# Graph-Machine-Learning-Group/sgp

Hardware: AMD Instinct MI355X
Metric: encoded node-steps/sec (higher is better)
Workload: dtype f32 (hop products: operands as fp16 hi + lo pairs, three 16-bit MFMA terms per product, fp32 accumulation -- agrees with fp32 to ~1e-7 of the operand scale; reservoir: recurrent products: state (|h| <= 1, x 2^14) and W_hh (per-row power-of-two scale) as two fp16 pieces (22 bits), hi*hi + hi*lo + lo*

## Files before the change

include/sgp_amd.h:

```cpp
#ifndef SGP_AMD_H
#define SGP_AMD_H

#include <stdint.h>

#ifdef __cplusplus
extern "C" {
#endif

#define SGP_ABI_VERSION 3

#define SGP_EINVAL   (-1)
#define SGP_EUNSUP   (-2)
#define SGP_ENOMEM   (-3)

#define SGP_ACT_TANH      0
#define SGP_ACT_RELU      1
#define SGP_ACT_SELF_NORM 2
#define SGP_ACT_IDENTITY  3
#define SGP_ACT_TANH_REL  4

typedef void* sgp_stream_t;

int sgp_abi_version(void);
const char* sgp_last_error(void);
// ... 8 lines not shown
                     float* Y, int64_t y_row_stride, int64_t y_batch_stride,
                     int32_t n_rows, int32_t n_cols, int32_t batch, int32_t feat,
                     const int32_t* pred, int32_t run_if, sgp_stream_t stream);

int sgp_spmm_tiled_f32(const int32_t* tile_row_ptr, const int32_t* uptr, const int32_t* ucol,
                       const int32_t* erow, const uint16_t* ecol, const float* eval,
                       int32_t tile_rows, int32_t n_tiles,
                       int32_t max_union, int32_t max_row_edges,
                       const float* X, int64_t x_row_stride, int64_t x_batch_stride,
                       const float* X_halo, int64_t xh_row_stride, int64_t xh_batch_stride,
                       int32_t n_own,
                       float* Y, int64_t y_row_stride, int64_t y_batch_stride,
                       int32_t n_rows, int32_t n_cols, int32_t batch, int32_t feat,
                       const int32_t* pred, int32_t run_if, sgp_stream_t stream);
int sgp_spmm_res_f32(const int32_t* uptr, const int32_t* ucol, const int32_t* usplit,
                     const int32_t* gptr, const int32_t* gsup, const int32_t* gidx, const float* gw,
                     const int32_t* rowmap,
                     int32_t n_tiles, int32_t max_union, int32_t max_tile_quads,
                     const float* X, int64_t x_row_stride, int64_t x_batch_stride,
                     const float* X_halo, int64_t xh_row_stride, int64_t xh_batch_stride,
                     int32_t n_own,
                     float* Y, int64_t y_row_stride, int64_t y_batch_stride,
                     int32_t n_rows, int32_t n_cols, int32_t batch, int32_t feat,
                     const int32_t* pred, int32_t run_if, sgp_stream_t stream);
int32_t sgp_spmm_res_max_union(void);
int32_t sgp_spmm_res_max_quads(void);
int sgp_spmm_res_tune(int32_t cfg);

int sgp_spmm_mix_f32(const int32_t* uptr, const int32_t* ucol, const int32_t* usplit,
                     const int32_t* gptr, const int32_t* gsup, const int32_t* gidx, const float* gw,
                     const int32_t* rowmap,
                     const int32_t* dptr, const int32_t* didx, const float* dw,
                     int32_t n_tiles, int32_t max_union, int32_t max_dense,
                     const float* X, int64_t x_row_stride, int64_t x_batch_stride,
                     const float* X_halo, int64_t xh_row_stride, int64_t xh_batch_stride,
                     int32_t n_own,
                     float* Y, int64_t y_row_stride, int64_t y_batch_stride,
                     int32_t n_rows, int32_t n_cols, int32_t batch, int32_t feat,
                     const int32_t* pred, int32_t run_if, sgp_stream_t stream);
int32_t sgp_spmm_mix_max_union(void);
int32_t sgp_spmm_mix_max_dense(int32_t halo);

int sgp_abs_max_f32(const float* X, int64_t x_row_stride, int64_t x_batch_stride,
                    int32_t n_rows, int32_t batch, int32_t feat, float* out, sgp_stream_t stream);


int sgp_col_stats_f32(const float* X, int64_t x_row_stride, int64_t x_batch_stride,
                      int32_t n_rows, int32_t batch, int32_t feat, int32_t t_stride, int32_t r_stride, int32_t accumulate,
                      float* stats, sgp_stream_t stream);

int sgp_split_prepare_f32(const float* stats, double n_samples, double s_eff, int32_t full,
                          const float* bound_in, float bound_scalar, float norm_inf, int32_t feat,
                          float* x_tab, float* bound_out, int32_t* flag, sgp_stream_t stream);

int sgp_spmm_split_f32(const int32_t* hdr, const int32_t* rowid, const int32_t* ucol, const void* afr,
                       const int32_t* adr, const float* rinv, int32_t n_tiles,
                       const float* X, int64_t x_row_stride, int64_t x_batch_stride,
                       const float* X_halo, int64_t xh_row_stride, int64_t xh_batch_stride, int32_t n_own,
                       float* Y, int64_t y_row_stride, int64_t y_batch_stride,
                       int32_t n_rows, int32_t n_cols, int32_t batch, int32_t feat,
                       const float* x_tab, int32_t accumulate, int32_t t_chunk, const int32_t* pred, int32_t run_if, sgp_stream_t stream);
int32_t sgp_spmm_split_chunks(void);
int32_t sgp_spmm_split_max_union(void);
int32_t sgp_spmm_split_waves(void);
int32_t sgp_spmm_split_rows_per_wave(void);
int32_t sgp_spmm_split_max_feat(void);

int sgp_spmm_split_banded_f32(const int32_t* hdr, const int32_t* rowid, const int32_t* ucol, const void* afr,
                              const int32_t* adr, const float* rinv, int32_t n_tiles,
                              const float* X, int64_t x_row_stride, int64_t x_batch_stride,
                              const float* X_halo, int64_t xh_row_stride, int64_t xh_batch_stride, int32_t n_own,
                              float* Y, int64_t y_row_stride, int64_t y_batch_stride,
                              int32_t n_rows, int32_t n_cols, int32_t batch, int32_t feat,
                              const float* x_tab, int32_t accumulate, int32_t t_chunk,
                              int32_t walk, const int32_t* band_first, int32_t n_bands,
                              const int32_t* pred, int32_t run_if, sgp_stream_t stream);

int sgp_spmm_split_wide_f32(const int32_t* hdr, const int32_t* rowid, const int32_t* ucol, const void* afr,
                            const int32_t* adr, const float* rinv, int32_t n_tiles,
                            const float* X, int64_t x_row_stride, int64_t x_batch_stride,
                            const float* X_halo, int64_t xh_row_stride, int64_t xh_batch_stride, int32_t n_own,
                            float* Y, int64_t y_row_stride, int64_t y_batch_stride,
                            int32_t n_rows, int32_t n_cols, int32_t batch, int32_t feat,
                            const float* x_tab, int32_t accumulate, int32_t t_chunk, const int32_t* pred, int32_t run_if, sgp_stream_t stream);
int sgp_spmm_split_wide_banded_f32(const int32_t* hdr, const int32_t* rowid, const int32_t* ucol, const void* afr,
                                   const int32_t* adr, const float* rinv, int32_t n_tiles,
                                   const float* X, int64_t x_row_stride, int64_t x_batch_stride,
                                   const float* X_halo, int64_t xh_row_stride, int64_t xh_batch_stride, int32_t n_own,
                                   float* Y, int64_t y_row_stride, int64_t y_batch_stride,
                                   int32_t n_rows, int32_t n_cols, int32_t batch, int32_t feat,
                                   const float* x_tab, int32_t accumulate, int32_t t_chunk,
                                   int32_t walk, const int32_t* band_first, int32_t n_bands,
                                   const int32_t* pred, int32_t run_if, sgp_stream_t stream);
int32_t sgp_spmm_split_wide_chunks(void);
int32_t sgp_spmm_split_wide_max_union(void);
int32_t sgp_spmm_split_wide_waves(void);
int32_t sgp_spmm_split_wide_rows_per_wave(void);
int32_t sgp_spmm_split_wide_max_feat(void);

int64_t sgp_split_plan_deal(const int64_t* rowptr, const int64_t* col, int64_t nnz, int64_t n_rows, int64_t n_cols,
                            const int64_t* order, int64_t n_order,
                            int32_t waves, int32_t chunks, int32_t max_union, int32_t rows_per_wave,
                            int64_t* wave_of_row, int64_t* slot_of_row, int64_t* tile_of_wave, int64_t* rows_of_wave);
int sgp_split_plan_fill(const int64_t* rowptr, const int64_t* col, const float* val, int64_t nnz, int64_t n_rows, int64_t n_cols,
                        const int64_t* wave_of_row, const int64_t* slot_of_row, const int64_t* tile_of_wave,
                        const int64_t* rows_of_wave, int64_t n_waves, int64_t n_tiles,
// ... 366 lines not shown
```

sgp_amd/csrc/split_prepare.hip:

```cpp
#include "common.h"

namespace {

__global__ __launch_bounds__(256) void col_stats_kernel(const float* x, long long xrs, long long xbs, int n_rows,
                                                        int t_stride, int feat, unsigned* amax, float* ssq) {
    const int q = feat >> 2;
    const int rpi = 256 / q;
    const int r0 = threadIdx.x / q, c = threadIdx.x - r0 * q;
    const float* xb = x + (long long)blockIdx.y * t_stride * xbs;
    unsigned m[4] = {0, 0, 0, 0};
    float s[4] = {0.f, 0.f, 0.f, 0.f};
    if (r0 < rpi) {
        auto take = [&](const float4 v) {
            m[0] = max(m[0], __float_as_uint(fabsf(v.x))); s[0] = fmaf(v.x, v.x, s[0]);
            m[1] = max(m[1], __float_as_uint(fabsf(v.y))); s[1] = fmaf(v.y, v.y, s[1]);
            m[2] = max(m[2], __float_as_uint(fabsf(v.z))); s[2] = fmaf(v.z, v.z, s[2]);
            m[3] = max(m[3], __float_as_uint(fabsf(v.w))); s[3] = fmaf(v.w, v.w, s[3]);
        };
        const long long step = (long long)gridDim.x * rpi;
        long long r = (long long)blockIdx.x * rpi + r0;
        for (; r + 3 * step < n_rows; r += 4 * step) {
            const float4 v0 = *(const float4*)(xb + r * xrs + 4 * c);
            const float4 v1 = *(const float4*)(xb + (r + step) * xrs + 4 * c);
            const float4 v2 = *(const float4*)(xb + (r + 2 * step) * xrs + 4 * c);
            const float4 v3 = *(const float4*)(xb + (r + 3 * step) * xrs + 4 * c);
            take(v0); take(v1); take(v2); take(v3);
        }
        for (; r < n_rows; r += step) take(*(const float4*)(xb + r * xrs + 4 * c));
    }
    __shared__ unsigned pm[256][4];
    __shared__ float ps[256][4];
#pragma unroll
    for (int i = 0; i < 4; ++i) { pm[threadIdx.x][i] = m[i]; ps[threadIdx.x][i] = s[i]; }
    __syncthreads();
    if (threadIdx.x < q) {
        for (int r = 1; r < rpi; ++r) {
#pragma unroll
            for (int i = 0; i < 4; ++i) { m[i] = max(m[i], pm[r * q + c][i]); s[i] += ps[r * q + c][i]; }
        }
#pragma unroll
        for (int i = 0; i < 4; ++i) { atomicMax(amax + 4 * c + i, m[i]); atomicAdd(ssq + 4 * c + i, s[i]); }
    }
}

struct PrepArgs {
    const unsigned* amax; const float* ssq;
    double n_samples, s_eff;
    int full;
    const float* bound_in; float bound_scalar;
    float norm_inf;
    int feat;
    float* tab; float* bound_out; int* flag;
};

__global__ __launch_bounds__(256) void split_prepare_kernel(PrepArgs a) {
    int ok = 1;
    for (int c = threadIdx.x; c < a.feat; c += 256) {
        float b;
        const float mx = a.amax ? __uint_as_float(a.amax[c]) : 0.f;
        if (a.bound_in) b = a.bound_in[c];
        else if (a.bound_scalar > 0.f) b = a.bound_scalar;
        else b = mx;
        if (a.amax && !(mx <= b)) ok = 0;
        float scale = 1.f, inv = 1.f;
        if (!(b >= 0.f) || !(b < __builtin_inff())) { ok = 0; b = __builtin_inff(); }
        else if (b > 0.f) {
            int k;
            const float mant = frexpf(b, &k);
            int e = (mant == 0.5f ? 15 : 14) - k;
            e = min(126, max(-126, e));
            scale = ldexpf(1.f, e); inv = ldexpf(1.f, -e);
            if (a.amax) {
                const double rms = sqrt((double)a.ssq[c] / a.n_samples);
                if (!((double)b * sqrt(a.s_eff) <= 65536.0 * rms)) ok = 0;
            }
        }
        a.tab[c] = scale; a.tab[a.feat + c] = inv;
        if (a.bound_out) a.bound_out[c] = b * a.norm_inf * (1.f + 1e-6f);
    }
    ok = __syncthreads_and(ok);
    if (threadIdx.x == 0) a.flag[0] = ok;
}

}

extern "C" {

int sgp_col_stats_f32(const float* X, int64_t x_row_stride, int64_t x_batch_stride,
                      int32_t n_rows, int32_t batch, int32_t feat, int32_t t_stride, int32_t r_stride, int32_t accumulate,
                      float* stats, sgp_stream_t stream) {
    SGP_REQUIRE(X && stats, "sgp_col_stats_f32: null pointer");
    SGP_REQUIRE(n_rows >= 0 && batch >= 0 && feat > 0 && feat % 4 == 0 && feat <= 1024 && t_stride >= 1 && r_stride >= 1,
                "sgp_col_stats_f32: feat must be a multiple of 4 up to 1024, strides >= 1");
    n_rows = (n_rows + r_stride - 1) / r_stride;
    x_row_stride *= r_stride;
    SGP_REQUIRE(sgp::aligned16(X) && x_row_stride % 4 == 0 && x_batch_stride % 4 == 0, "sgp_col_stats_f32: rows must be 16-byte aligned");
    hipStream_t s = (hipStream_t)stream;
    if (!accumulate) {
        hipError_t e = hipMemsetAsync(stats, 0, 2 * (size_t)feat * sizeof(float), s);
        if (e != hipSuccess) return sgp::fail((int)e, "sgp_col_stats_f32: memset: %s", hipGetErrorString(e));
    }
    if (n_rows == 0 || batch == 0) return 0;
    const int ns = (batch + t_stride - 1) / t_stride;
    SGP_REQUIRE(ns <= 65535, "sgp_col_stats_f32: more than 65535 sampled steps");
    const int rpi = 256 / (feat / 4);
    long long gx = ((long long)n_rows + rpi - 1) / rpi;
    const long long cap = 512 / ns > 0 ? 512 / ns : 1;
    if (gx > cap) gx = cap;
    hipLaunchKernelGGL(col_stats_kernel, dim3((unsigned)gx, (unsigned)ns), dim3(256), 0, s,
                       X, (long long)x_row_stride, (long long)x_batch_stride, n_rows, t_stride, feat,
                       (unsigned*)stats, stats + feat);
    return sgp::check_launch("col_stats");
}

int sgp_split_prepare_f32(const float* stats, double n_samples, double s_eff, int32_t full,
                          const float* bound_in, float bound_scalar, float norm_inf, int32_t feat,
                          float* x_tab, float* bound_out, int32_t* flag, sgp_stream_t stream) {
    SGP_REQUIRE(x_tab && flag, "sgp_split_prepare_f32: null pointer");
    SGP_REQUIRE(feat > 0 && feat <= 1024, "sgp_split_prepare_f32: feat out of range");
    SGP_REQUIRE(stats || bound_in || bound_scalar > 0.f, "sgp_split_prepare_f32: neither statistics nor a bound");
    SGP_REQUIRE(!stats || (n_samples >= 1.0 && s_eff >= 1.0), "sgp_split_prepare_f32: statistics need their sample counts");
    SGP_REQUIRE(stats || full == 0, "sgp_split_prepare_f32: full = 1 needs statistics");
    SGP_REQUIRE(bound_in || bound_scalar > 0.f || full, "sgp_split_prepare_f32: a measured bound needs statistics of every row");
    PrepArgs a;
    a.amax = (const unsigned*)stats; a.ssq = stats ? stats + feat : nullptr;
    a.n_samples = n_samples; a.s_eff = s_eff; a.full = full;
    a.bound_in = bound_in; a.bound_scalar = bound_scalar; a.norm_inf = norm_inf; a.feat = feat;
    a.tab = x_tab; a.bound_out = bound_out; a.flag = flag;
    hipLaunchKernelGGL(split_prepare_kernel, dim3(1), dim3(256), 0, (hipStream_t)stream, a);
    return sgp::check_launch("split_prepare");
}

}
```

sgp_amd/csrc/spmm.hip:

```cpp
#include "common.h"
#include <stdlib.h>

using sgp::f32x4;

namespace {

constexpr int kWave = 64;

__device__ __forceinline__ f32x4 ld4(const float* p) { return *reinterpret_cast<const f32x4*>(p); }
__device__ __forceinline__ void st4(float* p, f32x4 v) { *reinterpret_cast<f32x4*>(p) = v; }

struct Src {
    const float* x;  long long xrs, xbs;
    const float* xh; long long xhrs, xhbs;
    int n_own;
    const int* pred; int pred_want;
    __device__ __forceinline__ bool skip() const { return pred != nullptr && pred[0] != pred_want; }
    __device__ __forceinline__ const float* row(int b, int c) const {
        return (c < n_own) ? x + (long long)b * xbs + (long long)c * xrs
                           : xh + (long long)b * xhbs + (long long)(c - n_own) * xhrs;
    }
};

template <int LPR, int TB>
// ... 12 lines not shown
    for (int i = 0; i < TB; ++i) acc[i] = f32x4{0.f, 0.f, 0.f, 0.f};

    const int e1 = rowptr[row + 1];
    for (int e = rowptr[row] + g; e < e1; e += G) {
        const int c = col[e];
        const float v = val[e];
#pragma unroll
        for (int i = 0; i < TB; ++i) {
            if (fok && b0 + i < batch) {
                const f32x4 xv = ld4(src.row(b0 + i, c) + f0);
                acc[i] += v * xv;
            }
        }
    }
#pragma unroll
    for (int i = 0; i < TB; ++i) {
#pragma unroll
        for (int off = LPR; off < kWave; off <<= 1) {
            acc[i].x += __shfl_xor(acc[i].x, off);
            acc[i].y += __shfl_xor(acc[i].y, off);
            acc[i].z += __shfl_xor(acc[i].z, off);
            acc[i].w += __shfl_xor(acc[i].w, off);
        }
    }
#pragma unroll
    for (int i = 0; i < TB; ++i) {
        if (fok && b0 + i < batch && g == (i % G))
            st4(Y + (long long)(b0 + i) * ybs + (long long)row * yrs + f0, acc[i]);
    }
}

template <int LPR, int TB>
__global__ __launch_bounds__(256) void spmm_csr_rows(
        const int* __restrict__ rowptr, const int* __restrict__ col, const float* __restrict__ val,
        Src src, float* __restrict__ Y, long long yrs, long long ybs,
        int n_rows, int batch, int feat) {
    const int row = blockIdx.x * 4 + (threadIdx.x >> 6);
    if (row >= n_rows || src.skip()) return;
    csr_rows_body<LPR, TB>(rowptr, col, val, src, Y, yrs, ybs, batch, feat, row, blockIdx.y * TB);
}

template <int LPR, int TB>
__global__ __launch_bounds__(256) void spmm_csr_rows_strided(
        const int* __restrict__ rowptr, const int* __restrict__ col, const float* __restrict__ val,
        Src src, float* __restrict__ Y, long long yrs, long long ybs,
        int n_rows, int batch, int feat) {
    if (src.skip()) return;
    const int n_rb = (n_rows + 3) / 4, n_bb = (batch + TB - 1) / TB;
    for (int bb = blockIdx.y; bb < n_bb; bb += gridDim.y)
        for (int rb = blockIdx.x; rb < n_rb; rb += gridDim.x) {
            const int row = rb * 4 + (threadIdx.x >> 6);
            if (row < n_rows) csr_rows_body<LPR, TB>(rowptr, col, val, src, Y, yrs, ybs, batch, feat, row, bb * TB);
        }
}

__global__ __launch_bounds__(256) void spmm_csr_scalar(
        const int* __restrict__ rowptr, const int* __restrict__ col, const float* __restrict__ val,
        Src src, float* __restrict__ Y, long long yrs, long long ybs,
        int n_rows, int batch, int feat) {
    const int lane = threadIdx.x & 63;
    const int row = blockIdx.x * 4 + (threadIdx.x >> 6);
    const int b = blockIdx.y;
    if (row >= n_rows || src.skip()) return;
    const int e0 = rowptr[row], e1 = rowptr[row + 1];
    for (int f = lane; f < feat; f += kWave) {
        float acc = 0.f;
        for (int e = e0; e < e1; ++e) acc += val[e] * src.row(b, col[e])[f];
        Y[(long long)b * ybs + (long long)row * yrs + f] = acc;
    }
}

template <int S>
__device__ __forceinline__ int ror_i(int v) {
    if constexpr (S == 0) return v;
    else return __builtin_amdgcn_update_dpp(0, v, 0x120 + S, 0xf, 0xf, true);
}
template <int S>
__device__ __forceinline__ float ror_f(float v) {
    return __int_as_float(ror_i<S>(__float_as_int(v)));
}

template <int S0>
__device__ __forceinline__ void edge_half(const char* lds, int off, float w, int li16, f32x4& acc) {
    int ad[8];
    float wv[8];
    f32x4 xv[8];
#define SGP_ROT(i) ad[i] = ror_i<S0 + i>(off) + li16; wv[i] = ror_f<S0 + i>(w);
    SGP_ROT(0) SGP_ROT(1) SGP_ROT(2) SGP_ROT(3) SGP_ROT(4) SGP_ROT(5) SGP_ROT(6) SGP_ROT(7)
#undef SGP_ROT
#pragma unroll
    for (int i = 0; i < 8; ++i) xv[i] = *reinterpret_cast<const f32x4*>(lds + ad[i]);
#pragma unroll
    for (int i = 0; i < 8; ++i) acc += wv[i] * xv[i];
}

#define SGP_FMAC_ROR(S, ACC, W, X)                                                              \
    asm("v_fmac_f32_dpp %0, %1, %2 row_ror:" #S " row_mask:0xf bank_mask:0xf" : "+v"(ACC) : "v"(W), "v"(X))
#define SGP_STEP_ROR(S, I)                                                                      \
    SGP_FMAC_ROR(S, acc.x, w, xv[I].x); SGP_FMAC_ROR(S, acc.y, w, xv[I].y);                     \
    SGP_FMAC_ROR(S, acc.z, w, xv[I].z); SGP_FMAC_ROR(S, acc.w, w, xv[I].w);
template <int S0, int ABL = 0>
__device__ __forceinline__ void edge_half_dpp(const char* lds, int off, float w, int li16, f32x4& acc) {
    int ad[8];
    f32x4 xv[8];
#define SGP_ROT(i) ad[i] = ror_i<S0 + i>(off) + li16;
    SGP_ROT(0) SGP_ROT(1) SGP_ROT(2) SGP_ROT(3) SGP_ROT(4) SGP_ROT(5) SGP_ROT(6) SGP_ROT(7)
// ... 265 lines not shown
int sgp_spmm_tiled_form(int32_t tile_rows, int32_t max_row_edges, int32_t* rows_per_group, int32_t* batches) {
    SGP_REQUIRE(tile_rows > 0 && max_row_edges >= 0 && max_row_edges % 16 == 0, "sgp_spmm_tiled_form: bad size");
    if (tile_rows > sgp_spmm_tiled_max_tile_rows() || max_row_edges > sgp_spmm_tiled_max_row_edges())
        return sgp::fail(SGP_EUNSUP, "sgp_spmm_tiled_f32: tile_rows=%d / max_row_edges=%d out of range",
                         tile_rows, max_row_edges);
    int rpg = (tile_rows + kTiledGroups - 1) / kTiledGroups;
    rpg = rpg <= 2 ? rpg : (rpg <= 4 ? 4 : 6);
    const int nb = (rpg > 2 && max_row_edges <= 16) ? 1 : (max_row_edges <= 32 ? 2 : 8);
    if (rows_per_group) *rows_per_group = rpg;
    if (batches) *batches = nb;
    if (nb == 8 && rpg != 1)
        return sgp::fail(SGP_EUNSUP, "spmm_tiled: no kernel for rows/group=%d batches=%d", rpg, nb);
    return 0;
}

int32_t sgp_spmm_csr_form(int32_t feat, int32_t aligned, int32_t predicated) {
    (void)predicated;
    if (feat <= 0 || feat % 4 != 0 || !aligned) return 0;
    if (feat >= 256 || feat % 256 == 0) return 64;
    return feat > 64 ? 32 : feat > 32 ? 16 : feat > 16 ? 8 : 4;
}

int sgp_spmm_csr_f32(const int32_t* rowptr, const int32_t* col, const float* val,
                     const float* X, int64_t xrs, int64_t xbs,
                     const float* Xh, int64_t xhrs, int64_t xhbs, int32_t n_own,
                     float* Y, int64_t yrs, int64_t ybs,
                     int32_t n_rows, int32_t n_cols, int32_t batch, int32_t feat,
                     const int32_t* pred, int32_t run_if, sgp_stream_t stream) {
    const sgp::Predicate pr{pred, run_if};
    SGP_REQUIRE(rowptr && col && val && X && Y, "sgp_spmm_csr_f32: null pointer");
    SGP_REQUIRE(n_rows >= 0 && n_cols >= 0 && batch >= 0 && feat >= 0, "sgp_spmm_csr_f32: negative size");
    SGP_REQUIRE(Xh != nullptr || n_own >= n_cols, "sgp_spmm_csr_f32: n_own < n_cols needs X_halo");
    if (n_rows == 0 || batch == 0 || feat == 0) return 0;
    hipStream_t s = (hipStream_t)stream;
    Src src{X, xrs, xbs, Xh ? Xh : X, xhrs, xhbs, Xh ? n_own : 0x7fffffff, pr.flag, pr.want};
    const bool vec = feat % 4 == 0 && xrs % 4 == 0 && xbs % 4 == 0 && yrs % 4 == 0 && ybs % 4 == 0 &&
                     sgp::aligned16(X) && sgp::aligned16(Y) &&
                     (!Xh || (xhrs % 4 == 0 && xhbs % 4 == 0 && sgp::aligned16(Xh)));
    const unsigned gx = (n_rows + 3) / 4;
    if (sgp_spmm_csr_form(feat, vec, pr.flag != nullptr) == 0) {
        SGP_REQUIRE(batch <= 65535, "sgp_spmm_csr_f32: scalar path supports batch <= 65535");
        hipLaunchKernelGGL(spmm_csr_scalar, dim3(gx, batch), dim3(256), 0, s,
                           rowptr, col, val, src, Y, yrs, ybs, n_rows, batch, feat);
        return sgp::check_launch("spmm_csr_scalar");
    }
    constexpr int TB = 4;
    const unsigned gy = (batch + TB - 1) / TB;
    SGP_REQUIRE(gy <= 65535, "sgp_spmm_csr_f32: batch too large for one launch (chunk it)");
    const bool bounded = pr.flag != nullptr;
#define SGP_ROWS(LPR)                                                                          \
    do {                                                                                       \
        if (bounded)                                                                           \
            hipLaunchKernelGGL((spmm_csr_rows_strided<LPR, TB>),                               \
                               dim3(gx < 2048u ? gx : 2048u, gy < 8u ? gy : 8u, (feat + 4 * LPR - 1) / (4 * LPR)), \
                               dim3(256), 0, s, rowptr, col, val, src, Y, yrs, ybs, n_rows, batch, feat);          \
        else                                                                                   \
            hipLaunchKernelGGL((spmm_csr_rows<LPR, TB>), dim3(gx, gy, (feat + 4 * LPR - 1) / (4 * LPR)), \
                               dim3(256), 0, s, rowptr, col, val, src, Y, yrs, ybs, n_rows, batch, feat);  \
    } while (0)
    switch (sgp_spmm_csr_form(feat, 1, bounded)) {
        case 64: SGP_ROWS(64); break;
        case 32: SGP_ROWS(32); break;
        case 16: SGP_ROWS(16); break;
        case 8: SGP_ROWS(8); break;
        default: SGP_ROWS(4); break;
    }
#undef SGP_ROWS
    return sgp::check_launch("spmm_csr_rows");
}

int sgp_spmm_tiled_f32(const int32_t* trow, const int32_t* uptr, const int32_t* ucol,
                       const int32_t* erow, const uint16_t* ecol, const float* eval,
                       int32_t tile_rows, int32_t n_tiles, int32_t max_union, int32_t max_row_edges,
                       const float* X, int64_t xrs, int64_t xbs,
                       const float* Xh, int64_t xhrs, int64_t xhbs, int32_t n_own,
                       float* Y, int64_t yrs, int64_t ybs,
                       int32_t n_rows, int32_t n_cols, int32_t batch, int32_t feat,
                       const int32_t* pred, int32_t run_if, sgp_stream_t stream) {
    const sgp::Predicate pr{pred, run_if};
    SGP_REQUIRE(trow && uptr && ucol && erow && ecol && eval && X && Y, "sgp_spmm_tiled_f32: null pointer");
    SGP_REQUIRE(tile_rows > 0 && n_tiles >= 0 && n_rows >= 0 && batch >= 0 && max_union >= 0 &&
                max_row_edges >= 0 && max_row_edges % 16 == 0, "sgp_spmm_tiled_f32: bad size");
    SGP_REQUIRE((long long)tile_rows * n_tiles >= n_rows, "sgp_spmm_tiled_f32: tiles do not cover rows");
    {
        const long long own = Xh ? n_own : n_cols, far = Xh ? n_cols - n_own : 0;
        SGP_REQUIRE(n_cols >= 0 && own >= 0 && far >= 0 && own * xrs < (1ll << 31) && far * xhrs < (1ll << 31),
                    "sgp_spmm_tiled_f32: row offsets exceed 32 bits (use sgp_spmm_csr_f32)");
    }
    if (n_rows == 0 || batch == 0 || feat == 0) return 0;
    if (feat % 64 != 0)
        return sgp::fail(SGP_EUNSUP, "sgp_spmm_tiled_f32: feat=%d is not a multiple of 64", feat);
    if (max_union > kTiledCapacity)
        return sgp::fail(SGP_EUNSUP, "sgp_spmm_tiled_f32: a tile references %d distinct rows, LDS stage holds %d",
                         max_union, kTiledCapacity);
    int32_t rpg = 0, nb = 0;
    const int form_rc = sgp_spmm_tiled_form(tile_rows, max_row_edges, &rpg, &nb);
    if (form_rc && rpg == 0) return form_rc;
    SGP_REQUIRE(xrs % 4 == 0 && xbs % 4 == 0 && yrs % 4 == 0 && ybs % 4 == 0 &&
                sgp::aligned16(X) && sgp::aligned16(Y) &&
                (!Xh || (xhrs % 4 == 0 && xhbs % 4 == 0 && sgp::aligned16(Xh))),
                "sgp_spmm_tiled_f32: strides/pointers must be 16-byte aligned");
    TiledArgs a;
    a.trow = trow; a.uptr = uptr; a.ucol = ucol; a.erow = erow; a.ecol = ecol; a.eval = eval;
    a.tile_rows = tile_rows; a.n_tiles = n_tiles;
    a.src = Src{X, xrs, xbs, Xh ? Xh : X, xhrs, xhbs, Xh ? n_own : 0x7fffffff, pr.flag, pr.want};
    a.Y = Y; a.yrs = yrs; a.ybs = ybs;
    a.n_rows = n_rows; a.batch = batch; a.feat = feat;
// ... 14 lines not shown
```

sgp_amd/hip.py:

```python
import ctypes
import json
import os
import subprocess

import torch

_CSRC = os.path.join(os.path.dirname(os.path.abspath(__file__)), "csrc")
LIB_PATH = os.environ.get("SGP_AMD_LIB") or os.path.join(_CSRC, "libsgp_amd.so")

c_i32, c_i64, c_f32, c_f64, c_p = (ctypes.c_int32, ctypes.c_int64,
                                   ctypes.c_float, ctypes.c_double,
                                   ctypes.c_void_p)
c_u64 = ctypes.c_uint64

SIGNATURES = {
    "sgp_abi_version": (ctypes.c_int, []),
    "sgp_last_error": (ctypes.c_char_p, []),
    "sgp_build_arch": (ctypes.c_char_p, []),
    "sgp_tune_value": (c_i64, [ctypes.c_char_p, c_i64]),
    "sgp_spmm_csr_f32": (ctypes.c_int, [c_p, c_p, c_p,
                                        c_p, c_i64, c_i64,
                                        c_p, c_i64, c_i64, c_i32,
                                        c_p, c_i64, c_i64,
                                        c_i32, c_i32, c_i32, c_i32, c_p, c_i32, c_p]),
# ... 54 lines not shown
                                               c_i32, c_i32, c_i32, c_i32, c_i32, c_p]),
    "sgp_reservoir_fused_sums_f32": (ctypes.c_int, [c_p, c_i64, c_i64,
                                                    c_p, c_p, c_p,
                                                    c_p, c_i32,
                                                    c_p, c_i64, c_i64,
                                                    c_p, c_p, c_p,
                                                    c_i32, c_i32, c_i32, c_i32, c_i32, c_p]),
    "sgp_reservoir_window_supported": (c_i32, [c_i32, c_i32, c_i32]),
    "sgp_reservoir_window_workspace_bytes": (c_i64, [c_i32, c_i32, c_i32, c_i32, c_i64]),
    "sgp_reservoir_window_f32": (ctypes.c_int, [c_p, c_i64, c_i64, c_i64, c_i32,
                                                c_p, c_i64, c_i64, c_i64, c_i32,
                                                c_p,
                                                c_p, c_p, c_p, c_p, c_i32,
                                                c_p, c_p, c_i64,
                                                c_p, c_i32,
                                                c_i32, c_i32, c_i32, c_i32, c_i32, c_p]),
    "sgp_gesn_workspace_bytes": (c_i64, [c_i32, c_i32, c_i32]),
    "sgp_gesn_tune": (ctypes.c_int, [c_i32]),
    "sgp_gesn_f32": (ctypes.c_int, [c_p, c_p, c_p, c_p, c_i64, c_i64, c_p, c_p, c_p, c_p, c_i32,
                                    c_p, c_i64, c_i64, c_p, c_p,
                                    c_i32, c_i32, c_i32, c_i32, c_i32, c_p]),
    "sgp_gemm_nt_f32": (ctypes.c_int, [c_p, c_i64, c_p, c_i64, c_p, c_p, c_i64,
                                       c_i32, c_i32, c_i32, c_p]),
    "sgp_gesn_update_f32": (ctypes.c_int, [c_p, c_p, c_p, c_p, c_p, c_p, c_f64, c_i32,
                                           c_p, c_p, c_i64, c_i32, c_i32, c_p]),
    "sgp_node_mean_bcast_f32": (ctypes.c_int, [c_p, c_i64, c_i64,
                                               c_p, c_i64, c_i64, c_p,
                                               c_i32, c_i32, c_i32, c_p]),
    "sgp_bcast_rows_f32": (ctypes.c_int, [c_p, c_f32, c_p, c_i64, c_i64,
                                          c_i32, c_i32, c_i32, c_p]),
    "sgp_copy_rows_f32": (ctypes.c_int, [c_p, c_i64, c_i64, c_p, c_i64, c_i64,
                                         c_i32, c_i32, c_i32, c_p]),
    "sgp_gather_rows_f32": (ctypes.c_int, [c_p, c_i64, c_i64, c_p, c_p, c_i32,
                                           c_p, c_i64, c_i64, c_i32, c_i32, c_p]),
    "sgp_grouped_linear_packed_floats": (c_i64, [c_i32, c_i32, c_i32]),
    "sgp_grouped_linear_pack_f32": (ctypes.c_int, [c_p, c_p, c_i32, c_i32, c_i32, c_p]),
    "sgp_grouped_linear_f32": (ctypes.c_int, [c_p, c_i64, c_i64, c_p, c_p, c_p, c_p, c_i32,
                                              c_p, c_i64, c_i32, c_i32, c_i32, c_i32, c_p]),
    "sgp_grouped_linear_fwd_f32": (ctypes.c_int, [c_p, c_i64, c_i64, c_p, c_p, c_p, c_p, c_i32,
                                                  c_p, c_i64, c_p, c_f64, c_u64,
                                                  c_i32, c_i32, c_i32, c_i32, c_p]),
    "sgp_grouped_linear_dact_f32": (ctypes.c_int, [c_p, c_i64, c_p, c_i32, c_f64, c_u64, c_p, c_i64, c_i32, c_p]),
    "sgp_grouped_linear_transpose_f32": (ctypes.c_int, [c_p, c_p, c_i32, c_i32, c_i32, c_p]),
    "sgp_grouped_linear_wgrad_f32": (ctypes.c_int, [c_p, c_i64, c_i64, c_p, c_p, c_p, c_p,
                                                    c_i32, c_i32, c_i32, c_i32, c_p]),
    "sgp_grouped_linear_form": (ctypes.c_int, [c_i32, c_i32, c_i64, c_i64, c_i32, c_p, c_p]),
    "sgp_grouped_linear_wgrad_form": (ctypes.c_int, [c_i32, c_i32, c_i32, c_i32, c_p, c_p]),
    "sgp_abs_max_f32": (ctypes.c_int, [c_p, c_i64, c_i64, c_i32, c_i32, c_i32, c_p, c_p]),
    "sgp_spmm_split_f32": (ctypes.c_int, [c_p, c_p, c_p, c_p, c_p, c_p, c_i32, c_p, c_i64, c_i64,
                                          c_p, c_i64, c_i64, c_i32, c_p, c_i64, c_i64,
                                          c_i32, c_i32, c_i32, c_i32, c_p, c_i32, c_i32, c_p, c_i32, c_p]),
    "sgp_col_stats_f32": (ctypes.c_int, [c_p, c_i64, c_i64, c_i32, c_i32, c_i32, c_i32, c_i32, c_i32, c_p, c_p]),
    "sgp_split_prepare_f32": (ctypes.c_int, [c_p, c_f64, c_f64, c_i32, c_p, c_f32, c_f32, c_i32, c_p, c_p, c_p, c_p]),
    "sgp_spmm_split_wide_f32": (ctypes.c_int, [c_p, c_p, c_p, c_p, c_p, c_p, c_i32, c_p, c_i64, c_i64,
                                               c_p, c_i64, c_i64, c_i32, c_p, c_i64, c_i64,
                                               c_i32, c_i32, c_i32, c_i32, c_p, c_i32, c_i32, c_p, c_i32, c_p]),
    "sgp_spmm_split_wide_chunks": (c_i32, []),
    "sgp_spmm_split_wide_max_union": (c_i32, []),
    "sgp_spmm_split_wide_waves": (c_i32, []),
    "sgp_spmm_split_wide_rows_per_wave": (c_i32, []),
    "sgp_spmm_split_wide_max_feat": (c_i32, []),
    "sgp_spmm_split_chunks": (c_i32, []),
    "sgp_spmm_split_max_union": (c_i32, []),
    "sgp_spmm_split_waves": (c_i32, []),
    "sgp_spmm_split_rows_per_wave": (c_i32, []),
    "sgp_spmm_split_max_feat": (c_i32, []),
    "sgp_split_plan_deal": (c_i64, [c_p, c_p, c_i64, c_i64, c_i64, c_p, c_i64, c_i32, c_i32, c_i32, c_i32, c_p, c_p, c_p, c_p]),
    "sgp_split_plan_fill": (ctypes.c_int, [c_p, c_p, c_p, c_i64, c_i64, c_i64, c_p, c_p, c_p, c_p, c_i64, c_i64,
                                           c_i32, c_i32, c_i32, c_p, c_p, c_p, c_p, c_p, c_p, c_p, c_i32]),
    "sgp_split_plan_bands": (c_i64, [c_p, c_i64, c_i32, c_i64, c_i64, c_p]),
    "sgp_spmm_split_banded_f32": (ctypes.c_int, [c_p, c_p, c_p, c_p, c_p, c_p, c_i32, c_p, c_i64, c_i64,
                                                 c_p, c_i64, c_i64, c_i32, c_p, c_i64, c_i64,
                                                 c_i32, c_i32, c_i32, c_i32, c_p, c_i32, c_i32, c_i32, c_p, c_i32,
                                                 c_p, c_i32, c_p]),
    "sgp_spmm_split_wide_banded_f32": (ctypes.c_int, [c_p, c_p, c_p, c_p, c_p, c_p, c_i32, c_p, c_i64, c_i64,
                                                      c_p, c_i64, c_i64, c_i32, c_p, c_i64, c_i64,
                                                      c_i32, c_i32, c_i32, c_i32, c_p, c_i32, c_i32, c_i32, c_p, c_i32,
                                                      c_p, c_i32, c_p]),
    "sgp_spmm_colblock_f32": (ctypes.c_int, [c_p, c_p, c_p, c_i32, c_i32, c_p, c_i64, c_i64,
                                             c_p, c_i64, c_i64, c_i32, c_p, c_i64, c_i64,
                                             c_i32, c_i32, c_i32, c_i32, c_p, c_i32, c_p]),
    "sgp_spmm_colblock_rows_cap": (c_i32, []),
    "sgp_spmm_colblock_round_pad": (c_i32, []),
    "sgp_ridge_workspace_bytes": (c_i64, [c_i32, c_i64, c_i32, c_i32]),
    "sgp_ridge_form": (ctypes.c_int, [c_i32, c_i64, c_i32, c_i32, c_p]),
    "sgp_ridge_colmeans_f32": (ctypes.c_int, [c_p, c_i32, c_p, c_i64, c_i64, c_p, c_p, c_i64, c_p]),
    "sgp_ridge_gram_f32": (ctypes.c_int, [c_p, c_i32, c_p, c_i64, c_i64, c_p, c_i32, c_p, c_i64, c_p, c_i64, c_p]),
    "sgp_ridge_predict_score_f32": (ctypes.c_int, [c_p, c_i32, c_p, c_i64, c_i64, c_p, c_p, c_i32, c_i32,
                                                   c_p, c_p, c_i64, c_p, c_i64, c_i64,
                                                   c_p, c_i64, c_i64, c_i64, c_p, c_p, c_p, c_i64, c_p]),
    "sgp_dense_packed_floats": (c_i64, [c_i32, c_i32]),
    "sgp_dense_pack_f32": (ctypes.c_int, [c_p, c_i64, c_i32, c_i32, c_i32, c_p, c_p]),
    "sgp_dense_f32": (ctypes.c_int, [c_p, c_i64, c_p, c_i64, c_p, c_p, c_i32, c_i32, c_i32,
                                     c_i32, c_i32, c_i32, c_p, c_i64, c_p, c_i64, c_f64, c_u64, c_i64,
                                     c_p, c_i64, c_p, c_p, c_p]),
    "sgp_dense_form": (ctypes.c_int, [c_i32, c_i32, c_i32, c_i64, c_i32, c_p, c_p]),
    "sgp_dense_wgrad_workspace_floats": (c_i64, [c_i64, c_i32, c_i32, c_i32]),
    "sgp_dense_wgrad_f32": (ctypes.c_int, [c_p, c_i64, c_p, c_i64, c_p, c_i64, c_i32, c_i32, c_i32,
                                           c_p, c_i64, c_p, c_p, c_i64, c_p]),
    "sgp_row_segsum_f32": (ctypes.c_int, [c_p, c_i64, c_i64, c_i32, c_p, c_p, c_i32, c_p, c_p]),
    "sgp_masked_mae_f32": (ctypes.c_int, [c_p, c_p, c_p, c_i64, c_i32, c_p, c_p, c_p]),
    "sgp_masked_mae_bwd_f32": (ctypes.c_int, [c_p, c_p, c_p, c_i64, c_i32, c_p, c_p, c_p, c_p]),
    "sgp_multi_sqnorm_f32": (ctypes.c_int, [c_p, c_i64, c_p, c_p, c_p, c_p, c_p]),
    "sgp_adam_step_f32": (ctypes.c_int, [c_p, c_i64, c_p, c_p, c_p, c_p, c_p, c_f64,
                                         c_f64, c_f64, c_f64, c_f64, c_f64, c_i64, c_i32, c_p]),
    "sgp_masked_metrics_workspace_doubles": (c_i64, [c_i64, c_i32, c_i64, c_i32]),
# ... 273 lines not shown
    xp, xrs, xbs = _view3(x, "x")
    out = torch.empty(1, dtype=torch.float32, device=x.device)
    _check(lib.sgp_abs_max_f32(xp, xrs, xbs, x.shape[1], x.shape[0], x.shape[2], out.data_ptr(), _stream(x)),
           "sgp_abs_max_f32")
    return float(out.item())


def mark_unit_bounded(state):
    state._sgp_unit_bounded = state._version
    return state


def is_unit_bounded(state):
    return state is not None and getattr(state, "_sgp_unit_bounded", None) == state._version


class ColumnBound:

    def __init__(self, tensor):
        self.tensor = tensor


class SplitProfile:

    def __init__(self, tab, flag, bound_out):
        self.tab, self.flag, self.bound_out = tab, flag, bound_out


def _pred(pred):
    if pred is None:
        return None, 0
    flag, run_if = pred
    if not (torch.is_tensor(flag) and flag.is_cuda and flag.dtype == torch.int32 and flag.numel() >= 1):
        raise ValueError("pred: expected (int32 CUDA tensor, run_if)")
    return flag.data_ptr(), int(run_if)


@_on_device
def col_stats(x, t_stride=1, stats=None, r_stride=1):
    lib = require_gpu()
    xp, xrs, xbs = _view3(x, "x")
    acc = stats is not None
    if stats is None:
        stats = torch.empty(2, x.shape[2], dtype=torch.float32, device=x.device)
    _check(lib.sgp_col_stats_f32(xp, xrs, xbs, x.shape[1], x.shape[0], x.shape[2], int(t_stride), int(r_stride), int(acc),
                                 stats.data_ptr(), _stream(x)), "sgp_col_stats_f32")
    return stats


SPLIT_SAMPLE_STEPS = 8
SPLIT_SAMPLE_BYTES = 64 << 20


@_on_device
def split_profile(x, halo=None, bound=None, norm_inf=1.0, guard=True):
    import math
    lib = require_gpu()
    B, N, D = x.shape
    dev = x.device
    out = torch.empty(3 * D + 4, dtype=torch.float32, device=dev)
    tab, bound_out, flag = out[:2 * D].view(2, D), out[2 * D:3 * D], out[3 * D:3 * D + 1].view(torch.int32)
    if isinstance(bound, ColumnBound):
        b_in, b_scalar = bound.tensor, 0.0
        if b_in.numel() != D or b_in.device != dev:
            raise ValueError("ColumnBound does not match the operand")
    elif bound is None:
        b_in, b_scalar = None, 0.0
    else:
        b_in, b_scalar = None, float(bound)
        if not (b_scalar > 0 and math.isfinite(b_scalar)):
            raise ValueError("split_profile needs a finite positive bound on |x| (or None: measured)")
    measured = b_in is None and b_scalar == 0.0
    stats, n_samples, s_eff, full = None, 1.0, 1.0, 0
    if guard or measured:
        t_stride = 1 if measured else max(1, B // SPLIT_SAMPLE_STEPS)
        ns = -(-B // t_stride)
        r_stride = 1 if measured else max(1, -(-(ns * N * D * 4) // SPLIT_SAMPLE_BYTES))
        all_rows = N + (halo.shape[1] if halo is not None else 0)
        sources = [x] + ([halo] if halo is not None and halo.shape[1] > 0 else [])
        if measured or (t_stride == 1 and r_stride == 1):
            for k, src in enumerate(sources):
                stats = col_stats(src, 1, stats if k else None, r_stride=1)
            n_sum = float(B) * all_rows
        else:
            n_sum, first = 0.0, True
            if B > 1:
                ns = -(-(B - 1) // t_stride)
                for src in sources:
                    stats = col_stats(src[:B - 1], t_stride, None if first else stats, r_stride=r_stride)
                    first = False
                    n_sum += float(ns) * -(-src.shape[1] // r_stride)
            for src in sources:
                stats = col_stats(src[B - 1:], 1, None if first else stats, r_stride=1)
                first = False
                n_sum += float(src.shape[1])
        n_samples, s_eff, full = n_sum, (B * all_rows) / n_sum, int(t_stride == 1 and r_stride == 1)
    _check(lib.sgp_split_prepare_f32(None if stats is None else stats.data_ptr(), n_samples, s_eff, full,
                                     None if b_in is None else b_in.data_ptr(), b_scalar, float(norm_inf), D,
                                     tab.data_ptr(), bound_out.data_ptr(), flag.data_ptr(), _stream(x)),
           "sgp_split_prepare_f32")
    return SplitProfile(tab, flag, ColumnBound(bound_out))


_SPLIT_WALKS = {None: 0, "tile": 1, "time": 2}


@_on_device
def spmm_split(plan, x, y, profile, t_chunk=0, halo=None, n_own=None, predicated=False, walk=None):
    lib = require_gpu()
    ops, _ = _hop_operands(x, y, halo, n_own)
    if not isinstance(profile, SplitProfile):
        profile = split_profile(x, halo, profile, guard=False)
    plans = plan if isinstance(plan, (list, tuple)) else [plan]
    pr = _pred((profile.flag, 1) if predicated else None)
    for p in plans:
        entry = lib.sgp_spmm_split_wide_banded_f32 if p.afr.shape[1] == lib.sgp_spmm_split_wide_waves() and \
            p.afr.shape[2] == lib.sgp_spmm_split_wide_chunks() else lib.sgp_spmm_split_banded_f32
        if walk is None or isinstance(walk, str):
            how = (_SPLIT_WALKS[walk], None, 0)
        else:
            first, _ = p.band_table(walk)
            how = (3, first.data_ptr(), first.numel() - 1)
        _check(entry(
            p.hdr.data_ptr(), p.rowid.data_ptr(), p.ucol.data_ptr(), p.afr.data_ptr(), p.adr.data_ptr(),
            p.rinv.data_ptr(), p.n_tiles,
            *ops, p.n_rows, p.n_cols, x.shape[0], x.shape[2],
            profile.tab.data_ptr(), int(p.accumulate), t_chunk, *how, *pr, _stream(x)), "sgp_spmm_split_f32")
    return profile


@_on_device
def spmm_colblock(plan, x, y, halo=None, n_own=None, pred=None):
    lib = require_gpu()
    ops, _ = _hop_operands(x, y, halo, n_own)
    _check(lib.sgp_spmm_colblock_f32(
        plan.entries.data_ptr(), plan.segptr.data_ptr(), plan.wg_row0.data_ptr(), plan.n_wg, plan.n_blocks,
        *ops, plan.n_rows, plan.n_cols, x.shape[0], x.shape[2], *_pred(pred), _stream(x)), "sgp_spmm_colblock_f32")


def split_limits(wide=False):
    lib = load()
    if wide:
        return dict(waves=lib.sgp_spmm_split_wide_waves(), chunks=lib.sgp_spmm_split_wide_chunks(),
                    max_union=lib.sgp_spmm_split_wide_max_union(), rows_per_wave=lib.sgp_spmm_split_wide_rows_per_wave())
    return dict(waves=lib.sgp_spmm_split_waves(), chunks=lib.sgp_spmm_split_chunks(),
                max_union=lib.sgp_spmm_split_max_union(), rows_per_wave=lib.sgp_spmm_split_rows_per_wave())


def tiled_limits(feat):
    lib = load()
    return dict(max_union=min(lib.sgp_spmm_tiled_max_union(feat), lib.sgp_spmm_res_max_union()),
# ... 1293 lines not shown
```

Before: 1.317 billion.

## Fuse split admission stats and prepare into one last-block kernel

Adds a single-launch admission kernel that reads up to four strided segments, reduces column abs-max and sum of squares into replicated workspace slots, and has the last finishing block run the per-column prepare step and reset the workspace. It replaces a chain of memset, several col_stats launches and a prepare launch, cutting launch count and host overhead. It is selected only when the tune key 'admission' is 'fused'. The strided CSR launch grid is also capped by a total block budget that accounts for the z dimension.

```diff
diff --git a/include/sgp_amd.h b/include/sgp_amd.h
--- a/include/sgp_amd.h
+++ b/include/sgp_amd.h
@@ -84,6 +84,11 @@
 int sgp_split_prepare_f32(const float* stats, double n_samples, double s_eff, int32_t full,
                           const float* bound_in, float bound_scalar, float norm_inf, int32_t feat,
                           float* x_tab, float* bound_out, int32_t* flag, sgp_stream_t stream);
+
+int64_t sgp_split_admit_workspace_bytes(int32_t feat);
+int sgp_split_admit_f32(const int64_t* segs, int32_t n_segs, int32_t feat, double n_samples, double s_eff, int32_t full,
+                        const float* bound_in, float bound_scalar, float norm_inf,
+                        void* workspace, float* x_tab, float* bound_out, int32_t* flag, sgp_stream_t stream);
 
 int sgp_spmm_split_f32(const int32_t* hdr, const int32_t* rowid, const int32_t* ucol, const void* afr,
                        const int32_t* adr, const float* rinv, int32_t n_tiles,
diff --git a/sgp_amd/csrc/split_prepare.hip b/sgp_amd/csrc/split_prepare.hip
--- a/sgp_amd/csrc/split_prepare.hip
+++ b/sgp_amd/csrc/split_prepare.hip
@@ -53,33 +53,113 @@
     float* tab; float* bound_out; int* flag;
 };
 
+__device__ __forceinline__ int prepare_column(const PrepArgs& a, int c, float mx, float ssq) {
+    int ok = 1;
+    float b;
+    if (a.bound_in) b = a.bound_in[c];
+    else if (a.bound_scalar > 0.f) b = a.bound_scalar;
+    else b = mx;
+    if (a.amax && !(mx <= b)) ok = 0;
+    float scale = 1.f, inv = 1.f;
+    if (!(b >= 0.f) || !(b < __builtin_inff())) { ok = 0; b = __builtin_inff(); }
+    else if (b > 0.f) {
+        int k;
+        const float mant = frexpf(b, &k);
+        int e = (mant == 0.5f ? 15 : 14) - k;
+        e = min(126, max(-126, e));
+        scale = ldexpf(1.f, e); inv = ldexpf(1.f, -e);
+        if (a.amax) {
+            const double rms = sqrt((double)ssq / a.n_samples);
+            if (!((double)b * sqrt(a.s_eff) <= 65536.0 * rms)) ok = 0;
+        }
+    }
+    a.tab[c] = scale; a.tab[a.feat + c] = inv;
+    if (a.bound_out) a.bound_out[c] = b * a.norm_inf * (1.f + 1e-6f);
+    return ok;
+}
+
 __global__ __launch_bounds__(256) void split_prepare_kernel(PrepArgs a) {
     int ok = 1;
-    for (int c = threadIdx.x; c < a.feat; c += 256) {
-        float b;
-        const float mx = a.amax ? __uint_as_float(a.amax[c]) : 0.f;
-        if (a.bound_in) b = a.bound_in[c];
-        else if (a.bound_scalar > 0.f) b = a.bound_scalar;
-        else b = mx;
-        if (a.amax && !(mx <= b)) ok = 0;
-        float scale = 1.f, inv = 1.f;
-        if (!(b >= 0.f) || !(b < __builtin_inff())) { ok = 0; b = __builtin_inff(); }
-        else if (b > 0.f) {
-            int k;
-            const float mant = frexpf(b, &k);
-            int e = (mant == 0.5f ? 15 : 14) - k;
-            e = min(126, max(-126, e));
-            scale = ldexpf(1.f, e); inv = ldexpf(1.f, -e);
-            if (a.amax) {
-                const double rms = sqrt((double)a.ssq[c] / a.n_samples);
-                if (!((double)b * sqrt(a.s_eff) <= 65536.0 * rms)) ok = 0;
-            }
-        }
-        a.tab[c] = scale; a.tab[a.feat + c] = inv;
-        if (a.bound_out) a.bound_out[c] = b * a.norm_inf * (1.f + 1e-6f);
-    }
+    for (int c = threadIdx.x; c < a.feat; c += 256)
+        ok &= prepare_column(a, c, a.amax ? __uint_as_float(a.amax[c]) : 0.f, a.amax ? a.ssq[c] : 0.f);
     ok = __syncthreads_and(ok);
     if (threadIdx.x == 0) a.flag[0] = ok;
+}
+
+constexpr int kAdmitSegs = 4, kAdmitReplicas = 8, kAdmitHead = 64, kAdmitMaxGrid = 1024;
+
+struct AdmitSeg { const float* x; long long rs, bs; int n_rows, blocks, unit0; };
+struct AdmitArgs {
+    AdmitSeg seg[kAdmitSegs];
+    int n_segs, n_units;
+    unsigned* ws;
+    PrepArgs prep;
+};
+
+__global__ __launch_bounds__(256) void split_admit_kernel(AdmitArgs a) {
+    const int feat = a.prep.feat;
+    const int q = feat >> 2;
+    const int rpi = 256 / q;
+    const int r0 = threadIdx.x / q, c = threadIdx.x - r0 * q;
+    unsigned m[4] = {0, 0, 0, 0};
+    float s[4] = {0.f, 0.f, 0.f, 0.f};
+    if (r0 < rpi) {
+        for (int u = blockIdx.x; u < a.n_units; u += gridDim.x) {
+            AdmitSeg sg = a.seg[0];
+#pragma unroll
+            for (int k = 1; k < kAdmitSegs; ++k)
+                if (k < a.n_segs && u >= a.seg[k].unit0) sg = a.seg[k];
+            const int local = u - sg.unit0, step = local / sg.blocks, blk = local - step * sg.blocks;
+            const float* xb = sg.x + (long long)step * sg.bs + 4 * c;
+            const int row = blk * (4 * rpi) + r0;
+            float4 v[4];
+#pragma unroll
+            for (int i = 0; i < 4; ++i) {
+                const int r = row + i * rpi;
+                v[i] = r < sg.n_rows ? *(const float4*)(xb + (long long)r * sg.rs) : float4{0.f, 0.f, 0.f, 0.f};
+            }
+#pragma unroll
+            for (int i = 0; i < 4; ++i) {
+                m[0] = max(m[0], __float_as_uint(fabsf(v[i].x))); s[0] = fmaf(v[i].x, v[i].x, s[0]);
+                m[1] = max(m[1], __float_as_uint(fabsf(v[i].y))); s[1] = fmaf(v[i].y, v[i].y, s[1]);
+                m[2] = max(m[2], __float_as_uint(fabsf(v[i].z))); s[2] = fmaf(v[i].z, v[i].z, s[2]);
+                m[3] = max(m[3], __float_as_uint(fabsf(v[i].w))); s[3] = fmaf(v[i].w, v[i].w, s[3]);
+            }
+        }
+    }
+    __shared__ unsigned pm[256][4];
+    __shared__ float ps[256][4];
+    __shared__ int last;
+#pragma unroll
+    for (int i = 0; i < 4; ++i) { pm[threadIdx.x][i] = m[i]; ps[threadIdx.x][i] = s[i]; }
+    __syncthreads();
+    unsigned* rep = a.ws + kAdmitHead + (blockIdx.x % kAdmitReplicas) * 2 * feat;
+    for (int t = threadIdx.x; t < feat; t += 256) {
+        unsigned mv = 0;
+        float sv = 0.f;
+        for (int r = 0; r < rpi; ++r) { mv = max(mv, pm[r * q + (t >> 2)][t & 3]); sv += ps[r * q + (t >> 2)][t & 3]; }
+        atomicMax(rep + t, mv);
+        atomicAdd((float*)rep + feat + t, sv);
+    }
+    __threadfence();
+    __syncthreads();
+    if (threadIdx.x == 0) last = atomicAdd(a.ws, 1u) == gridDim.x - 1;
+    __syncthreads();
+    if (!last) return;
+    __threadfence();
+    int ok = 1;
+    for (int t = threadIdx.x; t < feat; t += 256) {
+        unsigned mv = 0;
+        float sv = 0.f;
+        for (int k = 0; k < kAdmitReplicas; ++k) {
+            unsigned* rk = a.ws + kAdmitHead + k * 2 * feat;
+            mv = max(mv, atomicExch(rk + t, 0u));
+            sv += __uint_as_float(atomicExch(rk + feat + t, 0u));
+        }
+        ok &= prepare_column(a.prep, t, __uint_as_float(mv), sv);
+    }
+    ok = __syncthreads_and(ok);
+    if (threadIdx.x == 0) { a.prep.flag[0] = ok; atomicExch(a.ws, 0u); }
 }
 
 }
@@ -131,4 +211,47 @@
     return sgp::check_launch("split_prepare");
 }
 
-}
+int64_t sgp_split_admit_workspace_bytes(int32_t feat) {
+    if (feat <= 0 || feat > 1024) return -1;
+    return (int64_t)(kAdmitHead + kAdmitReplicas * 2 * feat) * 4;
+}
+
+int sgp_split_admit_f32(const int64_t* segs, int32_t n_segs, int32_t feat, double n_samples, double s_eff, int32_t full,
+                        const float* bound_in, float bound_scalar, float norm_inf,
+                        void* workspace, float* x_tab, float* bound_out, int32_t* flag, sgp_stream_t stream) {
+    SGP_REQUIRE(segs && workspace && x_tab && flag, "sgp_split_admit_f32: null pointer");
+    SGP_REQUIRE(n_segs >= 1 && n_segs <= kAdmitSegs, "sgp_split_admit_f32: 1 .. 4 segments");
+    SGP_REQUIRE(feat > 0 && feat % 4 == 0 && feat <= 1024, "sgp_split_admit_f32: feat must be a multiple of 4 up to 1024");
+    SGP_REQUIRE(n_samples >= 1.0 && s_eff >= 1.0, "sgp_split_admit_f32: statistics need their sample counts");
+    SGP_REQUIRE(bound_in || bound_scalar > 0.f || full, "sgp_split_admit_f32: a measured bound needs statistics of every row");
+    SGP_REQUIRE(sgp::aligned16(workspace), "sgp_split_admit_f32: workspace must be 16-byte aligned");
+    AdmitArgs a;
+    const int rows_per_unit = 4 * (256 / (feat / 4));
+    long long units = 0;
+    for (int k = 0; k < kAdmitSegs; ++k) {
+        AdmitSeg& sg = a.seg[k];
+        if (k >= n_segs) { sg = AdmitSeg{nullptr, 0, 0, 0, 1, 0x7fffffff}; continue; }
+        const int64_t* d = segs + 5 * k;
+        const long long rows = d[3], steps = d[4];
+        SGP_REQUIRE(d[0] != 0 && rows >= 0 && steps >= 0 && rows <= 0x3fffffff && steps <= 0x3fffffff,
+                    "sgp_split_admit_f32: segment sizes out of range");
+        SGP_REQUIRE(d[0] % 16 == 0 && d[1] % 4 == 0 && d[2] % 4 == 0, "sgp_split_admit_f32: rows must be 16-byte aligned");
+        sg.x = (const float*)(uintptr_t)d[0]; sg.rs = d[1]; sg.bs = d[2]; sg.n_rows = (int)rows;
+        const long long blocks = (rows + rows_per_unit - 1) / rows_per_unit;
+        sg.blocks = blocks > 0 ? (int)blocks : 1;
+        sg.unit0 = (int)units;
+        units += blocks * steps;
+        SGP_REQUIRE(units < 0x7fffffff, "sgp_split_admit_f32: too many rows x steps for one launch");
+    }
+    a.n_segs = n_segs; a.n_units = (int)units; a.ws = (unsigned*)workspace;
+    PrepArgs& p = a.prep;
+    p.amax = a.ws; p.ssq = nullptr;
+    p.n_samples = n_samples; p.s_eff = s_eff; p.full = full;
+    p.bound_in = bound_in; p.bound_scalar = bound_scalar; p.norm_inf = norm_inf; p.feat = feat;
+    p.tab = x_tab; p.bound_out = bound_out; p.flag = flag;
+    const unsigned grid = units < 1 ? 1u : units < kAdmitMaxGrid ? (unsigned)units : (unsigned)kAdmitMaxGrid;
+    hipLaunchKernelGGL(split_admit_kernel, dim3(grid), dim3(256), 0, (hipStream_t)stream, a);
+    return sgp::check_launch("split_admit");
+}
+
+}
diff --git a/sgp_amd/csrc/spmm.hip b/sgp_amd/csrc/spmm.hip
--- a/sgp_amd/csrc/spmm.hip
+++ b/sgp_amd/csrc/spmm.hip
@@ -88,6 +88,14 @@
             const int row = rb * 4 + (threadIdx.x >> 6);
             if (row < n_rows) csr_rows_body<LPR, TB>(rowptr, col, val, src, Y, yrs, ybs, batch, feat, row, bb * TB);
         }
+}
+
+constexpr unsigned kStridedGrid = 2048;
+inline dim3 strided_grid(unsigned n_rb, unsigned n_bb, unsigned gz) {
+    const unsigned budget = kStridedGrid / gz > 0 ? kStridedGrid / gz : 1;
+    const unsigned gy = n_bb < 8u ? n_bb : 8u;
+    const unsigned cap = budget / gy > 0 ? budget / gy : 1;
+    return dim3(n_rb < cap ? n_rb : cap, gy, gz);
 }
 
 __global__ __launch_bounds__(256) void spmm_csr_scalar(
@@ -459,7 +467,7 @@
     do {                                                                                       \
         if (bounded)                                                                           \
             hipLaunchKernelGGL((spmm_csr_rows_strided<LPR, TB>),                               \
-                               dim3(gx < 2048u ? gx : 2048u, gy < 8u ? gy : 8u, (feat + 4 * LPR - 1) / (4 * LPR)), \
+                               strided_grid(gx, gy, (feat + 4 * LPR - 1) / (4 * LPR)),                             \
                                dim3(256), 0, s, rowptr, col, val, src, Y, yrs, ybs, n_rows, batch, feat);          \
         else                                                                                   \
             hipLaunchKernelGGL((spmm_csr_rows<LPR, TB>), dim3(gx, gy, (feat + 4 * LPR - 1) / (4 * LPR)), \
diff --git a/sgp_amd/hip.py b/sgp_amd/hip.py
--- a/sgp_amd/hip.py
+++ b/sgp_amd/hip.py
@@ -130,6 +130,8 @@
                                           c_i32, c_i32, c_i32, c_i32, c_p, c_i32, c_i32, c_p, c_i32, c_p]),
     "sgp_col_stats_f32": (ctypes.c_int, [c_p, c_i64, c_i64, c_i32, c_i32, c_i32, c_i32, c_i32, c_i32, c_p, c_p]),
     "sgp_split_prepare_f32": (ctypes.c_int, [c_p, c_f64, c_f64, c_i32, c_p, c_f32, c_f32, c_i32, c_p, c_p, c_p, c_p]),
+    "sgp_split_admit_workspace_bytes": (c_i64, [c_i32]),
+    "sgp_split_admit_f32": (ctypes.c_int, [c_p, c_i32, c_i32, c_f64, c_f64, c_i32, c_p, c_f32, c_f32, c_p, c_p, c_p, c_p, c_p]),
     "sgp_spmm_split_wide_f32": (ctypes.c_int, [c_p, c_p, c_p, c_p, c_p, c_p, c_i32, c_p, c_i64, c_i64,
                                                c_p, c_i64, c_i64, c_i32, c_p, c_i64, c_i64,
                                                c_i32, c_i32, c_i32, c_i32, c_p, c_i32, c_i32, c_p, c_i32, c_p]),
@@ -509,9 +511,22 @@
 SPLIT_SAMPLE_BYTES = 64 << 20
 
 
+_ADMIT_WORKSPACES = {}
+
+
+def _admit_workspace(device, feat):
+    key = (str(device), torch.cuda.current_stream(device).cuda_stream, feat)
+    ws = _ADMIT_WORKSPACES.get(key)
+    if ws is None:
+        ws = _ADMIT_WORKSPACES[key] = torch.zeros(load().sgp_split_admit_workspace_bytes(feat) // 4, dtype=torch.int32,
+                                                  device=device)
+    return ws
+
+
 @_on_device
 def split_profile(x, halo=None, bound=None, norm_inf=1.0, guard=True):
     import math
+    from . import tune
     lib = require_gpu()
     B, N, D = x.shape
     dev = x.device
@@ -529,6 +544,7 @@
             raise ValueError("split_profile needs a finite positive bound on |x| (or None: measured)")
     measured = b_in is None and b_scalar == 0.0
     stats, n_samples, s_eff, full = None, 1.0, 1.0, 0
+    samples = []
     if guard or measured:
         t_stride = 1 if measured else max(1, B // SPLIT_SAMPLE_STEPS)
         ns = -(-B // t_stride)
@@ -536,24 +552,27 @@
         all_rows = N + (halo.shape[1] if halo is not None else 0)
         sources = [x] + ([halo] if halo is not None and halo.shape[1] > 0 else [])
         if measured or (t_stride == 1 and r_stride == 1):
-            for k, src in enumerate(sources):
-                stats = col_stats(src, 1, stats if k else None, r_stride=1)
-            n_sum = float(B) * all_rows
+            samples = [(src, 1, 1) for src in sources]
         else:
-            n_sum, first = 0.0, True
             if B > 1:
-                ns = -(-(B - 1) // t_stride)
-                for src in sources:
-                    stats = col_stats(src[:B - 1], t_stride, None if first else stats, r_stride=r_stride)
-                    first = False
-                    n_sum += float(ns) * -(-src.shape[1] // r_stride)
-            for src in sources:
-                stats = col_stats(src[B - 1:], 1, None if first else stats, r_stride=1)
-                first = False
-                n_sum += float(src.shape[1])
+                samples = [(src[:B - 1], t_stride, r_stride) for src in sources]
+            samples += [(src[B - 1:], 1, 1) for src in sources]
+        n_sum = sum(float(-(-v.shape[0] // ts)) * -(-v.shape[1] // rs) for v, ts, rs in samples)
         n_samples, s_eff, full = n_sum, (B * all_rows) / n_sum, int(t_stride == 1 and r_stride == 1)
+    b_ptr = None if b_in is None else b_in.data_ptr()
+    if samples and tune.get("admission", "chain") == "fused":
+        segs = (ctypes.c_int64 * (5 * len(samples)))()
+        for k, (v, ts, rs) in enumerate(samples):
+            vp, vrs, vbs = _view3(v, "x")
+            segs[5 * k:5 * k + 5] = [vp, vrs * rs, vbs * ts, -(-v.shape[1] // rs), -(-v.shape[0] // ts)]
+        _check(lib.sgp_split_admit_f32(segs, len(samples), D, n_samples, s_eff, full, b_ptr, b_scalar, float(norm_inf),
+                                       _admit_workspace(dev, D).data_ptr(), tab.data_ptr(), bound_out.data_ptr(),
+                                       flag.data_ptr(), _stream(x)), "sgp_split_admit_f32")
+        return SplitProfile(tab, flag, ColumnBound(bound_out))
+    for k, (v, ts, rs) in enumerate(samples):
+        stats = col_stats(v, ts, stats if k else None, r_stride=rs)
     _check(lib.sgp_split_prepare_f32(None if stats is None else stats.data_ptr(), n_samples, s_eff, full,
-                                     None if b_in is None else b_in.data_ptr(), b_scalar, float(norm_inf), D,
+                                     b_ptr, b_scalar, float(norm_inf), D,
                                      tab.data_ptr(), bound_out.data_ptr(), flag.data_ptr(), _stream(x)),
            "sgp_split_prepare_f32")
     return SplitProfile(tab, flag, ColumnBound(bound_out))
```

Result: slower. 1.287 billion (-2.3%).
